# ajingu/RealSenseCalibration

Hardware: NVIDIA B200
Metric: LM iterations/sec (higher is better)
Workload: dtype f64

## Files before the change

realsensecalibration_b200/csrc/ba_cuda.cu:

```cuda
#include <dlfcn.h>

#include <algorithm>
#include <atomic>
#include <chrono>
#include <cmath>
#include <string>

#include "ba_dense.cuh"
#include "ba_dense_blocked.cuh"
#include "ba_kernels.cuh"
#include "ba_structure.cuh"
#include "ba_rcs.cuh"
#include "ba_fused_a.cuh"
#include "ba_strip_a.cuh"
#include "ba_exchange.cuh"
#include "ba_rig.cuh"

using namespace ba;

namespace {
typedef struct ncclComm* ncclComm_t;
struct NcclUniqueId { char internal[128]; };
struct Nccl {
  void* handle = nullptr;
// ... 479 lines not shown
  {
    FoldJob J = {{p->bp0.p, p->bp1.p, nullptr, nullptr}, {S_XE2, S_DE2, 0, 0}, {0, 0, 0, 0}};
    BA_LAUNCH(p, KT_FOLD, k_fold_multi, 2, 1024, 0, J, gce, p->scal.p);
  }
  BA_LAUNCH(p, KT_CANDIDATE, (k_candidate<6>), gcf, 256, 0, S.nf, p->f_act_ptr.p, p->xf.p, p->sf.p, p->yf.p, p->xf_c.p, p->bp0.p, p->bp1.p);
  {
    FoldJob J = {{p->bp0.p, p->bp1.p, nullptr, nullptr}, {S_XF2, S_DF2, 0, 0}, {0, 0, 0, 0}};
    BA_LAUNCH(p, KT_FOLD, k_fold_multi, 2, 1024, 0, J, gcf, p->scal.p);
  }
  BA_CUDA_TRY(cudaGetLastError());
  fam_end(p, F_UPDATE);
  fam_begin(p, F_COST);
  BA_TRY(run_cost_candidate(p));
  fam_end(p, F_COST);
  return allreduce_step_scalars(p);
}

FaParams fa_params(ba_cuda_problem* p, const ba_cuda_options& opt) {
  const Structure& S = p->S;
  FusedA& F = p->FA;
  const size_t nt = (size_t)F.n_tiles;
  FaParams P;
  P.tiles = F.tiles.p; P.e_ptr = S.e_ptr.p; P.ob_f = S.ob_f0.p; P.uv = p->uv.p;
  P.ob_meta = p->use_strip ? p->SA.ob_meta.p : F.ob_meta.p;
  P.tile_cams = p->use_strip ? p->SA.strip_cams.p : F.cams.group_target.p; P.cap = F.cap;
  P.pts_cap = F.pts_cap; P.tcam = F.tcam; P.tcs = F.tcs; P.pent_cap = F.pent_cap;
  P.pitem_begin = F.pairs.item_begin.p; P.pitem_end = F.pairs.item_end.p; P.pent = F.pairs.ent.p;
  P.citem_begin = F.cams.item_begin.p; P.citem_end = F.cams.item_end.p; P.cent = F.cams.ent.p;
  P.xe = p->xe.p; P.se = p->se.p; P.tab_f = p->tab_f.p; P.radius = p->scal.p + S_RADIUS;
  P.min_diag = opt.min_lm_diagonal; P.max_diag = opt.max_lm_diagonal;
  P.partP = F.partP.p; P.partC = F.partC.p; P.Lz = F.Lz.p; P.se_out = p->se.p;
  P.cost_partial = p->fa_part.p; P.g2_partial = p->fa_part.p + nt; P.gmax_partial = p->fa_part.p + 2 * nt;
  P.yf = p->yf.p; P.tabc_f = p->tabc_f.p; P.xe_c = p->xe_c.p;
  P.mcc_partial = p->fa_part.p + 3 * nt; P.x2_partial = p->fa_part.p + 4 * nt; P.d2_partial = p->fa_part.p + 5 * nt;
  P.cand_partial = p->fa_part.p + 6 * nt;
  P.RES = p->RES.p; P.JE = p->JE.p; P.JF = p->JF0.p;
  P.status = p->status.p;
  P.loss = p->loss;
  return P;
}

int fa_set_smem_attr(ba_cuda_problem* p) {
  if (!p->smem_attr_set) {
    const int kMax = (int)FA_SMEM_MAX;
    BA_CUDA_TRY(cudaFuncSetAttribute(k_fa_pass1<FA_FULL>, cudaFuncAttributeMaxDynamicSharedMemorySize, kMax));
    BA_CUDA_TRY(cudaFuncSetAttribute(k_fa_pass1<FA_NORMS>, cudaFuncAttributeMaxDynamicSharedMemorySize, kMax));
    BA_CUDA_TRY(cudaFuncSetAttribute(k_fa_pass1<FA_GRAD>, cudaFuncAttributeMaxDynamicSharedMemorySize, kMax));
    BA_CUDA_TRY(cudaFuncSetAttribute(k_fa_pass1<FA_FIRST>, cudaFuncAttributeMaxDynamicSharedMemorySize, kMax));
    BA_CUDA_TRY(cudaFuncSetAttribute(k_fa_pass2, cudaFuncAttributeMaxDynamicSharedMemorySize, kMax));
    BA_CUDA_TRY(cudaFuncSetAttribute(k_fa_jac, cudaFuncAttributeMaxDynamicSharedMemorySize, kMax));
    BA_CUDA_TRY(cudaFuncSetAttribute(k_sa_pass1<SA_FULL>, cudaFuncAttributeMaxDynamicSharedMemorySize, kMax));
    BA_CUDA_TRY(cudaFuncSetAttribute(k_sa_pass1<SA_GRAD>, cudaFuncAttributeMaxDynamicSharedMemorySize, kMax));
    BA_CUDA_TRY(cudaFuncSetAttribute(k_sa_pass1<SA_FIRST>, cudaFuncAttributeMaxDynamicSharedMemorySize, kMax));
    p->smem_attr_set = true;
  }
  return BA_OK;
}

int fa_reduce(ba_cuda_problem* p, bool cams, bool pairs) {
  const Structure& S = p->S;
  FusedA& F = p->FA;
  if (cams) {
    const ItemSet& I = F.cams;
    if (I.red_ch.n > 0)
      BA_LAUNCH(p, KT_FA_RED, (k_reduce_items<FA_NVC>), grid_for(I.red_ch.n, 4), 128, 0, I.red_ch.n, I.red_ch.ch, I.red_ch.seg.p, I.red_ch.begin.p,
                I.tgt_ptr.p, I.red_items.p, F.partC.p, F.red1C.p);
    BA_LAUNCH(p, KT_FA_RED, (k_reduce_final<FA_NVC>), grid_for(S.nf, 4), 128, 0, (int)S.nf, I.red_ch.seg_first.p, F.red1C.p, F.camacc.p);
  }
  if (pairs) {
    const ItemSet& I = F.pairs;
    if (I.red_ch.n > 0)
      BA_LAUNCH(p, KT_FA_RED, (k_reduce_items<36>), grid_for(I.red_ch.n, 4), 128, 0, I.red_ch.n, I.red_ch.ch, I.red_ch.seg.p, I.red_ch.begin.p,
                I.tgt_ptr.p, I.red_items.p, F.partP.p, F.red1P.p);
    BA_LAUNCH(p, KT_FA_RED, (k_reduce_final<36>), grid_for(S.ndest, 4), 128, 0, S.ndest, I.red_ch.seg_first.p, F.red1P.p, p->Pacc.p);
  }
  BA_CUDA_TRY(cudaGetLastError());
  return BA_OK;
}

int sa_linearize(ba_cuda_problem* p, const ba_cuda_options& opt, bool grad_only, bool first);

int fa_linearize(ba_cuda_problem* p, const ba_cuda_options& opt, bool norms, bool grad_only = false, bool first = false) {
  const Structure& S = p->S;
  FusedA& F = p->FA;
  BA_TRY(fa_set_smem_attr(p));
  if (p->use_strip) return sa_linearize(p, opt, grad_only, first);
  fam_begin(p, F_JAC);
  if (norms || first) {
    BA_LAUNCH(p, KT_MISC, k_fill, grid_for(S.nf * 6, 256), 256, 0, p->sf.p, S.nf * 6, 1.0);
    BA_LAUNCH(p, KT_MISC, k_fill, grid_for(S.ne * 3, 256), 256, 0, p->se.p, S.ne * 3, 1.0);
  }
  BA_TRY(build_tables(p, false));
  const FaParams P = fa_params(p, opt);
  const int nt = F.n_tiles;
  if (norms) {
    BA_LAUNCH(p, KT_FA_P1L, (k_fa_pass1<FA_NORMS>), nt, F.threads, F.smem1(), P);
    BA_TRY(fa_reduce(p, true, false));
    BA_TRY(allreduce(p, F.camacc.p, (size_t)S.nf * FA_NVC, kNcclSum));
    BA_LAUNCH(p, KT_MISC, (k_jacobi_scale<6, FA_NVC>), grid_for(S.nf * 6, 256), 256, 0, S.nf, F.camacc.p, p->sf.p);
    BA_CUDA_TRY(cudaGetLastError());
    fam_end(p, F_JAC);
    return BA_OK;
  }
  BA_CUDA_TRY(cudaMemsetAsync(p->status.p, 0, sizeof(int), p->st));
  if (grad_only) BA_LAUNCH(p, KT_FA_P1L, (k_fa_pass1<FA_GRAD>), nt, F.threads, F.smem1(), P);
  else if (first) BA_LAUNCH(p, KT_FA_P1, (k_fa_pass1<FA_FIRST>), nt, F.threads, F.smem1(), P);
// ... 124 lines not shown
  const double* radius = p->scal.p + S_RADIUS;
  const bool pcg = p->solver == BA_RCS_PCG;
  const bool sx = sx_active(p);
  fam_begin(p, F_SCHUR);
  if (pcg && sx) {
  } else if (pcg) {
    if (p->world > 1) BA_CUDA_TRY(cudaMemsetAsync(p->Sb.p, 0, p->Sb.bytes(), p->st));
    BA_LAUNCH(p, KT_ASSEMBLE, k_assemble_bsr, grid_for((int64_t)S.ndest * 36, 256), 256, 0, S.ndest, p->R.l2g.p, p->Pacc.p, nullptr, p->Sb.p);
  } else {
    BA_CUDA_TRY(cudaMemsetAsync(p->Sd.p, 0, sizeof(double) * n * n, p->st));
    BA_LAUNCH(p, KT_ASSEMBLE, k_assemble_dense, grid_for((int64_t)S.ndest * 36, 256), 256, 0, S.ndest, S.dest_fa.p, S.dest_fb.p, p->Pacc.p,
              nullptr, n, p->Sd.p);
  }
  fam_end(p, F_SCHUR);
  if (p->world > 1 && !(pcg && sx)) {
    fam_begin(p, F_COLL);
    if (pcg) BA_TRY(allreduce(p, p->Sb.p, (size_t)p->R.nd * 36, kNcclSum));
    else BA_TRY(allreduce(p, p->Sd.p, n * n, kNcclSum));
    fam_end(p, F_COLL);
  }
  fam_begin(p, F_SOLVE);
  if (pcg) {
    if (p->use_strip)
      BA_LAUNCH(p, KT_ASSEMBLE, k_sa_diag_rhs_bsr, grid_for(S.nf * 6, 128), 128, 0, S.nf, p->R.diag.p, F.camacc.p, radius, opt.min_lm_diagonal,
                opt.max_lm_diagonal, p->Sb.p, p->rhs.p);
    else
      BA_LAUNCH(p, KT_ASSEMBLE, k_diag_rhs_bsr, grid_for(S.nf * 6, 128), 128, 0, S.nf, p->R.diag.p, F.camacc.p, FA_NVC, F.camacc.p + 27, FA_NVC,
                radius, opt.min_lm_diagonal, opt.max_lm_diagonal, p->Sb.p, p->rhs.p);
    {
      LaunchScope scope(p, KT_RCS);
      BA_TRY(launch_pcg(p->pcg, p->R, p->Sb.p, p->rhs.p, p->yf.p, p->status.p, opt, p->st));
    }
    BA_CUDA_TRY(cudaMemcpyAsync(&p->h_pcg_iters, p->pcg.iters.p, sizeof(int), cudaMemcpyDeviceToHost, p->st));
  } else {
    if (p->use_strip)
      BA_LAUNCH(p, KT_ASSEMBLE, k_sa_diag_rhs_dense, grid_for(S.nf * 6, 128), 128, 0, S.nf, F.camacc.p, radius, opt.min_lm_diagonal,
                opt.max_lm_diagonal, n, p->Sd.p, p->rhs.p);
    else
      BA_LAUNCH(p, KT_ASSEMBLE, k_diag_rhs_dense, grid_for(S.nf * 6, 128), 128, 0, S.nf, F.camacc.p, FA_NVC, F.camacc.p + 27, FA_NVC, radius,
                opt.min_lm_diagonal, opt.max_lm_diagonal, n, p->Sd.p, p->rhs.p);
    LaunchScope scope(p, KT_RCS);
    BA_TRY(dense_solve(p, n));
  }
  fam_end(p, F_SOLVE);
  fam_begin(p, F_UPDATE);
  const int gcf = (int)grid_for(S.nf * 6, 256);
  BA_LAUNCH(p, KT_CANDIDATE, (k_candidate<6>), gcf, 256, 0, S.nf, p->f_act_ptr.p, p->xf.p, p->sf.p, p->yf.p, p->xf_c.p, p->bp0.p, p->bp1.p);
  {
    FoldJob J = {{p->bp0.p, p->bp1.p, nullptr, nullptr}, {S_XF2, S_DF2, 0, 0}, {0, 0, 0, 0}};
    BA_LAUNCH(p, KT_FOLD, k_fold_multi, 2, 1024, 0, J, gcf, p->scal.p);
  }
  BA_TRY(build_tables(p, true));
  const FaParams P = fa_params(p, opt);
  BA_LAUNCH(p, KT_FA_P2, k_fa_pass2, F.n_tiles, F.threads2, F.smem2(), P);
  {
    FoldJob J = {{P.mcc_partial, P.x2_partial, P.d2_partial, P.cand_partial}, {S_MCC, S_XE2, S_DE2, S_CAND}, {0, 0, 0, 0}};
    BA_LAUNCH(p, KT_FOLD, k_fold_multi, 4, 1024, 0, J, F.n_tiles, p->scal.p);
  }
  BA_CUDA_TRY(cudaGetLastError());
  fam_end(p, F_UPDATE);
  return allreduce_step_scalars(p);
}

bool lm_fused(const ba_cuda_problem* p) { return p->model == 0 && p->use_fused && !p->lm.opt.force_generic_path; }

int sx_prepare(ba_cuda_problem* p) {
  const Structure& S = p->S;
  SparseExchange& X = p->SX;
  X.on = false; X.world = p->world; X.nvc = p->use_strip ? SA_NVC : FA_NVC;
  if (!nccl().AllGather || !env_int("BA_SX", 0, 1, 1)) return BA_OK;
  cudaStream_t st = p->st;
  const int64_t nf = S.nf, nd = p->R.nd;
  DVec<int32_t> cflag, cpos, dflag, dpos;
  BA_TRY(cflag.alloc(nf + 1)); BA_TRY(cpos.alloc(nf + 1)); BA_TRY(dflag.alloc((size_t)S.ndest + 1)); BA_TRY(dpos.alloc((size_t)S.ndest + 1));
  BA_CUDA_TRY(cudaMemsetAsync(cflag.p, 0, sizeof(int32_t) * (nf + 1), st));
  BA_CUDA_TRY(cudaMemsetAsync(dflag.p, 0, sizeof(int32_t) * ((size_t)S.ndest + 1), st));
  k_sx_flags<<<grid_for(nf, 256), 256, 0, st>>>(S.fobs_ptr.p, nf, cflag.p);
  k_sx_send_flags<<<grid_for(S.ndest, 256), 256, 0, st>>>(S.ndest, S.dest_fa.p, S.dest_fb.p, cflag.p, dflag.p);
  BA_TRY(cub_call([&](void* t, size_t& b) { return cub::DeviceScan::ExclusiveSum(t, b, cflag.p, cpos.p, (int)(nf + 1), st); }));
  BA_TRY(cub_call([&](void* t, size_t& b) { return cub::DeviceScan::ExclusiveSum(t, b, dflag.p, dpos.p, S.ndest + 1, st); }));
  int32_t h2[2] = {0, 0};
  BA_CUDA_TRY(cudaMemcpyAsync(&h2[0], cpos.p + nf, sizeof(int32_t), cudaMemcpyDeviceToHost, st));
  BA_CUDA_TRY(cudaMemcpyAsync(&h2[1], dpos.p + S.ndest, sizeof(int32_t), cudaMemcpyDeviceToHost, st));
  BA_CUDA_TRY(cudaStreamSynchronize(st));
  X.nc_local = h2[0]; X.n_send = h2[1];
  BA_TRY(X.my_cams.alloc((size_t)X.nc_local)); BA_TRY(X.send_d.alloc((size_t)X.n_send));
  k_sx_compact<<<grid_for(nf, 256), 256, 0, st>>>(cflag.p, cpos.p, nf, X.my_cams.p);
  k_sx_compact<<<grid_for(S.ndest, 256), 256, 0, st>>>(dflag.p, dpos.p, S.ndest, X.send_d.p);
  DVec<int64_t> cnt;
  BA_TRY(cnt.alloc(2 * (size_t)p->world));
  const int64_t mine[2] = {X.n_send, X.nc_local};
  BA_CUDA_TRY(cudaMemcpyAsync(cnt.p + 2 * p->rank, mine, sizeof(mine), cudaMemcpyHostToDevice, st));
  int rc = nccl().AllGather(cnt.p + 2 * p->rank, cnt.p, 2, kNcclInt64, p->comm, st);
  if (rc != 0) return fail(BA_ERR_NCCL, "ncclAllGather failed (%d)", rc);
  std::vector<int64_t> h(2 * (size_t)p->world);
  BA_CUDA_TRY(cudaMemcpyAsync(h.data(), cnt.p, sizeof(int64_t) * h.size(), cudaMemcpyDeviceToHost, st));
  BA_CUDA_TRY(cudaStreamSynchronize(st));
  int64_t sum_nd = 0, max_nd = 1, max_nc = 1;
  for (int r = 0; r < p->world; ++r) { sum_nd += h[2 * r]; max_nd = std::max(max_nd, h[2 * r]); max_nc = std::max(max_nc, h[2 * r + 1]); }
  if ((double)max_nd * p->world > 1.5 * (double)nd) return BA_OK;
  X.max_nd = (int)max_nd; X.max_nc = (int)max_nc;
  X.slot = (size_t)max_nd * 36 + (size_t)max_nc * X.nvc + 4;
  DVec<int32_t> lists_d, lists_c;
  BA_TRY(lists_d.alloc((size_t)max_nd * p->world)); BA_TRY(lists_c.alloc((size_t)max_nc * p->world));
  BA_CUDA_TRY(cudaMemsetAsync(lists_d.p, 0xff, sizeof(int32_t) * (size_t)max_nd * p->world, st));
  BA_CUDA_TRY(cudaMemsetAsync(lists_c.p, 0xff, sizeof(int32_t) * (size_t)max_nc * p->world, st));
  k_sx_gather_l2g<<<grid_for(X.n_send, 256), 256, 0, st>>>(X.n_send, X.send_d.p, p->R.l2g.p, lists_d.p + (size_t)max_nd * p->rank);
  BA_CUDA_TRY(cudaMemcpyAsync(lists_c.p + (size_t)max_nc * p->rank, X.my_cams.p, sizeof(int32_t) * X.nc_local, cudaMemcpyDeviceToDevice, st));
  rc = nccl().AllGather(lists_d.p + (size_t)max_nd * p->rank, lists_d.p, (size_t)max_nd, kNcclInt32, p->comm, st);
  if (rc == 0) rc = nccl().AllGather(lists_c.p + (size_t)max_nc * p->rank, lists_c.p, (size_t)max_nc, kNcclInt32, p->comm, st);
// ... 1307 lines not shown
```

realsensecalibration_b200/csrc/ba_fused_a.cuh:

```cuda
#pragma once
#include <cuda_pipeline.h>

#include <chrono>
#include <cstdio>

#include "ba_kernels.cuh"
#include "ba_structure.cuh"

namespace ba {

constexpr int FA_TOBS_DEFAULT = 256;
constexpr int FA_KMAX = 64;
constexpr int FA_TPTS = 4096;
constexpr int FA_TCAM = 48;
constexpr int FA_CH_PAIR = 16;
constexpr int FA_CH_RED = 64;
constexpr int FA_NVC = 33;
constexpr int FA_MAX_THREADS = 512;
constexpr int FA_THREADS_DEFAULT = 128;
constexpr int FA_REC = 22;
constexpr int FA_REC2 = 10;
constexpr int FA_PENT_MAX = 6144;
constexpr size_t FA_SMEM_MAX = 231000;
constexpr int FA_LS = 10;
// ... 427 lines not shown
                                                          sb, keys.p, vals.p);
      L.lap("pair fill (32-bit keys)");
      D.mode = 1; D.sb = sb; D.key_bits = 2 * sb + tb;
      D.tile_cam_ptr = F.cams.tile_group_ptr.p; D.tile_cams = F.cams.group_target.p;
      D.dh_keys = S.dh_keys.p; D.dh_val = S.dh_val.p; D.dh_mask = S.dh_mask; D.dh_shift = S.dh_shift;
      BA_TRY(build_items<uint32_t>(F.pairs, keys, vals, np, F.n_tiles, S.ndest, F.ch_pair, true, D, st));
    } else {
      DVec<uint64_t> keys;
      BA_TRY(keys.alloc(np));
      k_fa_pair_fill<<<grid_for(ne, 128), 128, 0, st>>>(S.e_ptr.p, S.ob_f0.p, ne, nf, off.p, tile_of_pt.p, F.tile_pt_ptr.p, S.dest_keys.p,
                                                        S.ndest, S.dh_keys.n ? S.dh_keys.p : nullptr, S.dh_val.p, S.dh_mask, S.dh_shift, keys.p,
                                                        vals.p);
      L.lap("pair fill");
      D.key_bits = bits_for((uint64_t)F.n_tiles * (uint64_t)S.ndest);
      BA_TRY(build_items<uint64_t>(F.pairs, keys, vals, np, F.n_tiles, S.ndest, F.ch_pair, true, D, st));
    }
  }
  {
    const int nt = F.n_tiles;
    BA_TRY(F.tile_pent_ptr.alloc((size_t)nt + 1)); BA_TRY(F.tile_cent_ptr.alloc((size_t)nt + 1));
    k_fa_tile_ent_ptr<<<grid_for(nt + 1, 256), 256, 0, st>>>(nt, F.pairs.tile_group_ptr.p, F.pairs.group_ptr.p, F.tile_pent_ptr.p);
    k_fa_tile_ent_ptr<<<grid_for(nt + 1, 256), 256, 0, st>>>(nt, F.cams.tile_group_ptr.p, F.cams.group_ptr.p, F.tile_cent_ptr.p);
    DVec<int> stat;
    BA_TRY(stat.alloc_zero(3, st));
    k_fa_tile_stats<<<grid_for(nt, 256), 256, 0, st>>>(nt, F.tile_pt_ptr.p, F.cams.tile_group_ptr.p, F.tile_pent_ptr.p, stat.p);
    int h[3] = {0, 0, 0};
    BA_CUDA_TRY(cudaMemcpyAsync(h, stat.p, sizeof(h), cudaMemcpyDeviceToHost, st));
    BA_CUDA_TRY(cudaStreamSynchronize(st));
    F.pts_cap = std::max(1, std::min(h[0], FA_TPTS));
    F.tcam = std::max(1, std::min(h[1], FA_TCAM));
    F.tcs = F.tcam | 1;
    F.pent_cap = std::min(h[2], FA_PENT_MAX);
    F.pent_cap += F.pent_cap & 1;
    if (F.smem1() > FA_SMEM_MAX) {
      const size_t excess = (F.smem1() - FA_SMEM_MAX + 7) / 8 * 2;
      F.pent_cap = (size_t)F.pent_cap > excess ? F.pent_cap - (int)excess : 0;
    }
    if (F.smem1() > FA_SMEM_MAX || F.smem2() > FA_SMEM_MAX || F.smemj(FA_JAC_THREADS) > FA_SMEM_MAX) return BA_ERR_UNSUPPORTED;
  }
  L.lap("pair items, geometry");
  BA_TRY(F.tiles.alloc((size_t)F.n_tiles));
  k_fa_tile_desc<<<grid_for(F.n_tiles, 256), 256, 0, st>>>(F.n_tiles, F.tile_pt_ptr.p, S.e_ptr.p, F.cams.tile_group_ptr.p, F.tile_pent_ptr.p,
                                                          F.tile_cent_ptr.p, F.pairs.tile_item_ptr.p, F.cams.tile_item_ptr.p, F.tiles.p);
  BA_TRY(F.partP.alloc((size_t)F.pairs.n_items * 36)); BA_TRY(F.partC.alloc((size_t)F.cams.n_items * FA_NVC));
  BA_TRY(F.red1P.alloc((size_t)F.pairs.red_ch.n * 36)); BA_TRY(F.red1C.alloc((size_t)F.cams.red_ch.n * FA_NVC));
  BA_TRY(F.camacc.alloc((size_t)nf * FA_NVC + 2 + 64));
  BA_TRY(F.Lz.alloc((size_t)ne * 9));
  BA_CUDA_TRY(cudaStreamSynchronize(st));
  BA_CUDA_TRY(cudaGetLastError());
  F.ready = true;
  return BA_OK;
}

__device__ __forceinline__ void fa_linearize(const double* __restrict__ T, const double* X, const double* s, double2 ob, double* r,
                                             double* je, double* jf) {
  double q[3];
  mat3_vec(T, X, q);
  const double p0 = q[0] + T[18], p1 = q[1] + T[19], p2 = q[2] + T[20];
  r[0] = T[21] * p0 / p2 + T[23] - ob.x;
  r[1] = T[22] * p1 / p2 + T[24] - ob.y;
  const double iz = 1.0 / p2;
  const double a = T[21] * iz, bb = -T[21] * p0 * iz * iz, cc = T[22] * iz, dd = -T[22] * p1 * iz * iz;
  double D[9];
  rot_deriv(T + 9, T[25] != 0.0 ? X : q, D);
#pragma unroll
  for (int k = 0; k < 3; ++k) {
    jf[k] = (a * D[k] + bb * D[6 + k]) * T[26 + k];
    jf[6 + k] = (cc * D[3 + k] + dd * D[6 + k]) * T[26 + k];
  }
  jf[3] = a * T[29]; jf[4] = 0.0;        jf[5] = bb * T[31];
  jf[9] = 0.0;       jf[10] = cc * T[30]; jf[11] = dd * T[31];
  je[0] = (a * T[0] + bb * T[6]) * s[0]; je[1] = (a * T[1] + bb * T[7]) * s[1]; je[2] = (a * T[2] + bb * T[8]) * s[2];
  je[3] = (cc * T[3] + dd * T[6]) * s[0]; je[4] = (cc * T[4] + dd * T[7]) * s[1]; je[5] = (cc * T[5] + dd * T[8]) * s[2];
}

__device__ __forceinline__ bool fa_chol3(const double* M , double* Lp) {
  const double d0 = M[0];
  if (!(d0 > 0.0) || !isfinite(d0)) return false;
  const double i0 = rsqrt(d0);
  const double l10 = M[1] * i0, l20 = M[2] * i0;
  const double d1 = M[3] - l10 * l10;
  if (!(d1 > 0.0) || !isfinite(d1)) return false;
  const double i1 = rsqrt(d1);
  const double l21 = (M[4] - l20 * l10) * i1;
  const double d2 = M[5] - l20 * l20 - l21 * l21;
  if (!(d2 > 0.0) || !isfinite(d2)) return false;
  Lp[0] = l10; Lp[1] = l20; Lp[2] = l21; Lp[3] = i0; Lp[4] = i1; Lp[5] = rsqrt(d2);
  return true;
}
__device__ __forceinline__ void fa_fwd3(const double* Lp, double* x) {
  x[0] *= Lp[3];
  x[1] = (x[1] - Lp[0] * x[0]) * Lp[4];
  x[2] = (x[2] - Lp[1] * x[0] - Lp[2] * x[1]) * Lp[5];
}
__device__ __forceinline__ void fa_bwd3(const double* Lp, double* x) {
  x[2] *= Lp[5];
  x[1] = (x[1] - Lp[2] * x[2]) * Lp[4];
  x[0] = (x[0] - Lp[0] * x[1] - Lp[1] * x[2]) * Lp[3];
}

struct FaParams {
  const FaTile* tiles;
  const int64_t* e_ptr; const int32_t* ob_f; const uint32_t* ob_meta; const double2* uv;
  const int32_t* tile_cams;
  const int64_t* pitem_begin; const int64_t* pitem_end; const int32_t* pent;
  const int64_t* citem_begin; const int64_t* citem_end; const int32_t* cent;
  int cap, pts_cap, tcam, tcs, pent_cap;
  const double* xe; const double* se; const double* tab_f; const double* radius;
  double min_diag, max_diag;
  double* partP; double* partC; double* Lz; double* se_out;
  double* cost_partial; double* gmax_partial; double* g2_partial;
  const double* yf; const double* tabc_f; double* xe_c;
  double* mcc_partial; double* x2_partial; double* d2_partial; double* cand_partial;
  double* RES; double* JE; double* JF;
  int* status;
  LossSpec loss;
};

__device__ __forceinline__ double fa_apply_loss(const LossSpec L, double* r, double* je, double* jf) {
  const double s = r[0] * r[0] + r[1] * r[1];
  if (L.type == 0) return s;
  double rho, w;
  loss_apply(L, s, &rho, &w);
  r[0] *= w; r[1] *= w;
#pragma unroll
  for (int k = 0; k < 6; ++k) je[k] *= w;
// ... 593 lines not shown
```

realsensecalibration_b200/csrc/ba_strip_a.cuh:

```cuda
#pragma once
#include "ba_fused_a.cuh"

namespace ba {

constexpr int SA_NT = 512;
constexpr int SA_NCS_MAX = 64;
constexpr int SA_NVC = 39;
constexpr int SA_REC = 22;
constexpr int SA_NF_CAP = 1024;
constexpr int SA_POS_MAX = 4096;
constexpr int SA_CM_MAX = 8;
constexpr int SA_TYPE_IDLE = 0, SA_TYPE_PAIR = 1, SA_TYPE_FLUSH = 2, SA_TYPE_CAM = 3;
constexpr int SA_FULL = 0, SA_GRAD = 2, SA_FIRST = 3;

__host__ __device__ inline int sa_xs_len(int pts_cap) { return (3 * pts_cap + 4 + 1) & ~1; }

struct __align__(16) SaTile {
  int64_t pt0, ob0, pos0, ent0, pidx0, fout0;
  int32_t npts, nobs, npos, nent;
};
static_assert(sizeof(SaTile) == 64, "SaTile is loaded as four 16-byte words");
struct __align__(16) SaStrip {
  int64_t cam0, pout0, cout0;
  int32_t tile0, ntiles, ncs, nflush;
  int32_t flush_t0;
  int32_t npp, ncact, cbase;
};
static_assert(sizeof(SaStrip) == 64, "SaStrip");

struct StripA {
  bool ready = false;
  int n_tiles = 0, n_strips = 0, tobs = 0, L = 0, kmax = 0;
  int cap_pos = 0, pts_cap = 0, ncs_cap = 0, tcs = 0, ent_cap = 0, pidx_cap = 0, segw = 0, nobs_cap = 0;
  int64_t n_pout = 0, n_fout = 0, n_cout = 0;
  DVec<int64_t> tile_pt_ptr;
  DVec<SaTile> tiles;
  DVec<SaStrip> strips;
  DVec<int32_t> strip_cams;
  DVec<int64_t> strip_cam_ptr;
  DVec<uint32_t> slot_out;
  DVec<uint32_t> pm;
  DVec<double2> puv;
  DVec<uint16_t> pidx;
  DVec<int32_t> ent;
  DVec<uint16_t> seg;
  DVec<uint32_t> ob_meta;
  DVec<int32_t> red_items_p, red_items_c;
  DVec<int64_t> tgt_ptr_p, tgt_ptr_c;
  Chunks red_ch_p, red_ch_c;
  DVec<double> partP, partC, red1P, red1C;
  size_t smem() const {
    size_t b = ((size_t)cap_pos * SA_REC + (size_t)tcs * TAB + 2 * (size_t)sa_xs_len(pts_cap)) * 8;
    b += (size_t)cap_pos * 16 + (size_t)cap_pos * 4 + (size_t)pidx_cap * 2 + (size_t)ent_cap * 4 + (size_t)segw * 2 + 64;
    return b;
  }
};

__global__ void k_sa_strip_keys(int64_t nb, const int32_t* __restrict__ ob_e, const int32_t* __restrict__ ob_f,
                                const int32_t* __restrict__ tile_of_pt, int L, int64_t nf, uint64_t* __restrict__ keys) {
  const int64_t o = blockIdx.x * (int64_t)blockDim.x + threadIdx.x;
  if (o < nb) keys[o] = (uint64_t)(tile_of_pt[ob_e[o]] / L) * (uint64_t)nf + (uint64_t)ob_f[o];
}
__global__ void k_sa_split_keys(int ng, const uint64_t* __restrict__ ukeys, int64_t nf, int32_t* __restrict__ gstrip, int32_t* __restrict__ gcam) {
  const int g = blockIdx.x * blockDim.x + threadIdx.x;
  if (g >= ng) return;
  gstrip[g] = (int32_t)(ukeys[g] / (uint64_t)nf);
  gcam[g] = (int32_t)(ukeys[g] % (uint64_t)nf);
}
__global__ void k_sa_obs_slot(int64_t nb, const int32_t* __restrict__ ob_e, const int32_t* __restrict__ ob_f,
                              const int32_t* __restrict__ tile_of_pt, const int64_t* __restrict__ tile_pt_ptr, int L,
                              const int64_t* __restrict__ strip_cam_ptr, const int32_t* __restrict__ strip_cams,
                              uint8_t* __restrict__ ob_slot, uint32_t* __restrict__ ob_meta) {
  const int64_t o = blockIdx.x * (int64_t)blockDim.x + threadIdx.x;
  if (o >= nb) return;
  const int32_t e = ob_e[o], tile = tile_of_pt[e], strip = tile / L, cam = ob_f[o];
  int64_t lo = strip_cam_ptr[strip], hi = strip_cam_ptr[strip + 1];
  const int64_t c0 = lo;
  while (lo < hi) {
    const int64_t mid = (lo + hi) >> 1;
    if (strip_cams[mid] < cam) lo = mid + 1; else hi = mid;
  }
  const uint32_t slot = (uint32_t)min((int64_t)255, lo - c0);
  ob_slot[o] = (uint8_t)slot;
  ob_meta[o] = (uint32_t)(e - tile_pt_ptr[tile]) | (slot << 16);
}

__device__ __forceinline__ int sa_class(int ncs, int slot, int l) { return ncs >= 8 ? (slot & 7) : (l & 7); }
__device__ __forceinline__ int sa_class_rows(int nobs, int max_class) { return min(max_class, (nobs * 17 / 16 + 7) / 8); }

__global__ void __launch_bounds__(256)
k_sa_tile_sizes(int n_tiles, int L, const int64_t* __restrict__ tile_pt_ptr, const int64_t* __restrict__ e_ptr,
                const uint8_t* __restrict__ ob_slot, const int64_t* __restrict__ strip_cam_ptr, int64_t* __restrict__ tile_npos,
                int64_t* __restrict__ tile_nent, int64_t* __restrict__ tile_npidx, int* __restrict__ stat) {
  __shared__ int cls[8];
  __shared__ int npair, dup;
  const int t = blockIdx.x;
  if (threadIdx.x < 8) cls[threadIdx.x] = 0;
  if (threadIdx.x == 0) { npair = 0; dup = 0; }
  __syncthreads();
  const int64_t pt0 = tile_pt_ptr[t], pt1 = tile_pt_ptr[t + 1];
  const int64_t ob0 = e_ptr[pt0];
  const int nobs = (int)(e_ptr[pt1] - ob0), npts = (int)(pt1 - pt0);
  const int strip = t / L;
  const int ncs = (int)(strip_cam_ptr[strip + 1] - strip_cam_ptr[strip]);
  for (int l = threadIdx.x; l < nobs; l += blockDim.x) atomicAdd(&cls[sa_class(ncs, ob_slot[ob0 + l], l)], 1);
  for (int lp = threadIdx.x; lp < npts; lp += blockDim.x) {
    const int64_t b = e_ptr[pt0 + lp], n = e_ptr[pt0 + lp + 1];
// ... 662 lines not shown
  A.ent_cap = max_nent;
  if (A.smem() > FA_SMEM_MAX) {
    const size_t excess = (A.smem() - FA_SMEM_MAX + 15) / 16 * 4;
    if ((size_t)A.ent_cap <= excess) return BA_ERR_UNSUPPORTED;
    A.ent_cap = (int)(A.ent_cap - excess) & ~3;
    if (A.ent_cap < max_nent / 2) return BA_ERR_UNSUPPORTED;
  }
  BA_TRY(A.ent.alloc((size_t)tot[1] + 8)); BA_TRY(A.seg.alloc((size_t)nt * A.segw + 8));
  DVec<int64_t> t_nfl, fout0;
  BA_TRY(t_nfl.alloc_zero((size_t)nt + 1, st));
  {
    SaEntParams P;
    P.L = L; P.ncs_cap = A.ncs_cap; P.segw = A.segw; P.stage_cap = 12288;
    P.tiles = A.tiles.p; P.strips = A.strips.p; P.e_ptr = S.e_ptr.p; P.ob_e = S.ob_e.p; P.ob_slot = ob_slot.p; P.pidx = A.pidx.p;
    P.dslot = dslot.p; P.cslot = cslot.p; P.cthr = cthr.p; P.thr_of = thr_of.p; P.ent = A.ent.p; P.seg = A.seg.p; P.tile_nfl = t_nfl.p;
    const size_t sm = ((size_t)2 * A.segw + 1 + P.stage_cap) * sizeof(int);
    BA_CUDA_TRY(cudaFuncSetAttribute(k_sa_tile_entries, cudaFuncAttributeMaxDynamicSharedMemorySize, 100 * 1024));
    k_sa_tile_entries<<<nt, 512, sm, st>>>(P);
  }
  BA_TRY(sa_exclusive_scan(t_nfl, fout0, nt + 1, st));
  k_sa_set_fout<<<grid_for(nt, 256), 256, 0, st>>>(nt, fout0.p, A.tiles.p);
  BA_CUDA_TRY(cudaMemcpyAsync(&A.n_fout, fout0.p + nt, sizeof(int64_t), cudaMemcpyDeviceToHost, st));
  BA_CUDA_TRY(cudaStreamSynchronize(st));
  BA_CUDA_TRY(cudaGetLastError());
  Lp.lap("strip: entries");
  const int64_t n_pblocks = A.n_pout + A.n_fout;
  if (n_pblocks >= (int64_t)INT32_MAX / 64 || A.n_cout >= (int64_t)INT32_MAX / 64) return BA_ERR_UNSUPPORTED;
  {
    DVec<int32_t> ptarget, ctarget, iota;
    BA_TRY(ptarget.alloc((size_t)n_pblocks)); BA_TRY(ctarget.alloc((size_t)A.n_cout));
    k_sa_targets_persist<<<grid_for((int64_t)ns * SA_NT, 256), 256, 0, st>>>(ns, A.strips.p, A.slot_out.p, slot_dest.p, A.strip_cams.p, nf,
                                                                            S.dh_keys.p, S.dh_val.p, S.dh_mask, S.dh_shift, ptarget.p, ctarget.p);
    k_sa_targets_flush<<<grid_for(nt, 4), 128, 0, st>>>(nt, L, A.segw, nf_cap, A.tiles.p, A.strips.p, A.seg.p, fl_dest.p, A.strip_cams.p, nf,
                                                       S.dh_keys.p, S.dh_val.p, S.dh_mask, S.dh_shift, A.n_pout, ptarget.p);
    const int64_t nmax = std::max(n_pblocks, A.n_cout);
    BA_TRY(iota.alloc((size_t)nmax));
    k_iota<<<grid_for(nmax, 256), 256, 0, st>>>(iota.p, nmax, 0);
    BA_TRY(sort_to_csr(ptarget.p, iota.p, n_pblocks, S.ndest, A.tgt_ptr_p, A.red_items_p, st));
    BA_TRY(build_chunks(A.red_ch_p, A.tgt_ptr_p.p, S.ndest, FA_CH_RED, st));
    BA_TRY(sort_to_csr(ctarget.p, iota.p, A.n_cout, nf, A.tgt_ptr_c, A.red_items_c, st));
    BA_TRY(build_chunks(A.red_ch_c, A.tgt_ptr_c.p, (int)nf, FA_CH_RED, st));
    BA_CUDA_TRY(cudaStreamSynchronize(st));
  }
  Lp.lap("strip: reduction lists");
  BA_TRY(A.partP.alloc((size_t)n_pblocks * 36)); BA_TRY(A.partC.alloc((size_t)A.n_cout * SA_NVC));
  BA_TRY(A.red1P.alloc((size_t)A.red_ch_p.n * 36)); BA_TRY(A.red1C.alloc((size_t)A.red_ch_c.n * SA_NVC));
  F.n_tiles = nt; F.tobs = tobs; F.kmax = A.kmax; F.cap = std::max(A.nobs_cap, 1);
  F.threads = SA_NT; F.threads2 = env_int("BA_FA_THREADS2", 32, FA_MAX_THREADS, tobs >= 640 ? 256 : 128) / 32 * 32;
  F.pts_cap = A.pts_cap; F.tcam = std::min(A.ncs_cap, FA_TCAM); F.tcs = F.tcam | 1; F.pent_cap = 0;
  if (F.smem2() > FA_SMEM_MAX || F.smemj(FA_JAC_THREADS) > FA_SMEM_MAX) return BA_ERR_UNSUPPORTED;
  BA_TRY(F.tiles.alloc((size_t)nt));
  k_sa_fa_tiles<<<grid_for(nt, 256), 256, 0, st>>>(nt, L, A.tiles.p, A.strips.p, F.tiles.p);
  BA_TRY(F.camacc.alloc((size_t)nf * SA_NVC + 2 + 64));
  BA_TRY(F.Lz.alloc((size_t)ne * 9));
  BA_CUDA_TRY(cudaStreamSynchronize(st));
  BA_CUDA_TRY(cudaGetLastError());
  if (Lp.on)
    std::fprintf(stderr, "[ba_cuda timing]   strip geometry: tobs %d L %d tiles %d strips %d | positions %d points %d cameras %d entries staged %d of %d "
                         "owner slots %d | smem %zu B | blocks: %lld per strip + %lld flushed, %lld camera\n", tobs, L, nt, ns, A.cap_pos, A.pts_cap,
                 A.ncs_cap, A.ent_cap, max_nent, A.segw, A.smem(), (long long)A.n_pout, (long long)A.n_fout, (long long)A.n_cout);
  A.ready = true; F.ready = true;
  return BA_OK;
}

struct SaParams {
  const SaStrip* strips; const SaTile* tiles; const int32_t* strip_cams; const uint32_t* slot_out;
  const uint32_t* pm; const double2* puv; const uint16_t* pidx; const int32_t* ent; const uint16_t* seg;
  int segw, cap_pos, pts_cap, tcs, ent_cap, pidx_cap;
  const double* xe; const double* se; const double* tab_f; const double* radius;
  double min_diag, max_diag;
  double* partP; double* partC; int64_t n_pout;
  double* Lz; double* se_out; double* cost_partial; double* g2_partial; double* gmax_partial; int* status;
  int dbg;
  unsigned long long* clocks;
  LossSpec loss;
};

__device__ __forceinline__ uint32_t sa_smem_u32(const void* p) { return (uint32_t)__cvta_generic_to_shared(p); }
__device__ __forceinline__ void sa_mbar_init(uint64_t* bar, int count) {
  asm volatile("mbarrier.init.shared::cta.b64 [%0], %1;" ::"r"(sa_smem_u32(bar)), "r"(count) : "memory");
}
__device__ __forceinline__ void sa_mbar_expect_tx(uint64_t* bar, uint32_t bytes) {
  asm volatile("mbarrier.arrive.expect_tx.shared::cta.b64 _, [%0], %1;" ::"r"(sa_smem_u32(bar)), "r"(bytes) : "memory");
}
__device__ __forceinline__ void sa_mbar_wait(uint64_t* bar, uint32_t parity) {
  uint32_t ok = 0;
  const uint32_t a = sa_smem_u32(bar);
  do {
    asm volatile("{\n .reg .pred p;\n mbarrier.try_wait.parity.shared::cta.b64 p, [%1], %2;\n selp.u32 %0, 1, 0, p;\n}\n"
                 : "=r"(ok) : "r"(a), "r"(parity) : "memory");
  } while (!ok);
}
__device__ __forceinline__ void sa_bulk_g2s(void* dst, const void* src, uint32_t bytes, uint64_t* bar) {
  asm volatile("cp.async.bulk.shared::cluster.global.mbarrier::complete_tx::bytes [%0], [%1], %2, [%3];"
               ::"r"(sa_smem_u32(dst)), "l"(src), "r"(bytes), "r"(sa_smem_u32(bar)) : "memory");
}

template <int MODE>
__global__ void __launch_bounds__(SA_NT, 1) k_sa_pass1(SaParams P) {
  constexpr bool FIRST = MODE == SA_FIRST, FULL = MODE == SA_FULL || FIRST, UNIT = FIRST;
  extern __shared__ __align__(128) double smem[];
  double* rec = smem;
  double* tabs = rec + (size_t)P.cap_pos * SA_REC;
  double* xs = tabs + (size_t)P.tcs * TAB;
  double* ss = xs + sa_xs_len(P.pts_cap);
  double2* puv_s = reinterpret_cast<double2*>(ss + sa_xs_len(P.pts_cap));
  uint32_t* pm_s = reinterpret_cast<uint32_t*>(puv_s + P.cap_pos);
  uint16_t* pidx_s = reinterpret_cast<uint16_t*>(pm_s + P.cap_pos);
  int32_t* ent_s = reinterpret_cast<int32_t*>(pidx_s + P.pidx_cap);
  uint16_t* seg_s = reinterpret_cast<uint16_t*>(ent_s + P.ent_cap);
  uint64_t* bars = reinterpret_cast<uint64_t*>(seg_s + P.segw);
  __shared__ double red[96];
  const int tid = threadIdx.x, lane = tid & 31, warp = tid >> 5;
// ... 317 lines not shown
  const int64_t t = blockIdx.x * (int64_t)blockDim.x + threadIdx.x;
  if (t >= nf * SA_NVC) return;
  const int64_t c = t / SA_NVC;
  const int v = (int)(t % SA_NVC);
  double f;
  if (v < 21) {
    int a = 0, rem = v;
    while (rem >= 6 - a) { rem -= 6 - a; ++a; }
    f = sf[6 * c + a] * sf[6 * c + a + rem];
  } else if (v < 33) {
    f = sf[6 * c + (v - 21) % 6];
  } else {
    f = sf[6 * c + (v - 33)] * sf[6 * c + (v - 33)];
  }
  camacc[t] *= f;
}
__global__ void k_sa_jacobi_scale(int64_t nf, const double* __restrict__ camacc, double* __restrict__ sf) {
  const int64_t t = blockIdx.x * (int64_t)blockDim.x + threadIdx.x;
  if (t >= nf * 6) return;
  sf[t] = 1.0 / (1.0 + sqrt(camacc[(t / 6) * SA_NVC + 33 + (t % 6)]));
}
__global__ void k_sa_diag_rhs_bsr(int64_t nf, const int32_t* __restrict__ diag, const double* __restrict__ camacc, const double* __restrict__ radius_p,
                                  double min_diag, double max_diag, double* __restrict__ Sb, double* __restrict__ rhs) {
  const int64_t t = blockIdx.x * (int64_t)blockDim.x + threadIdx.x;
  if (t >= nf * 6) return;
  const int64_t f = t / 6;
  const int a = (int)(t % 6);
  const double* H = camacc + f * SA_NVC;
  double* B = Sb + (int64_t)diag[f] * 36;
#pragma unroll
  for (int b = 0; b < 6; ++b) {
    double h = H[a <= b ? sym_idx6(a, b) : sym_idx6(b, a)];
    if (a == b) { const double d = sqrt(fmin(fmax(H[33 + a], min_diag), max_diag) / *radius_p); h += d * d; }
    B[a * 6 + b] += h;
  }
  rhs[t] = H[21 + a] - H[27 + a];
}
__global__ void k_sa_diag_rhs_dense(int64_t nf, const double* __restrict__ camacc, const double* __restrict__ radius_p, double min_diag,
                                    double max_diag, int64_t n, double* __restrict__ Sd, double* __restrict__ rhs) {
  const int64_t t = blockIdx.x * (int64_t)blockDim.x + threadIdx.x;
  if (t >= nf * 6) return;
  const int64_t f = t / 6;
  const int a = (int)(t % 6);
  const double* H = camacc + f * SA_NVC;
#pragma unroll
  for (int b = 0; b < 6; ++b) {
    double h = H[a <= b ? sym_idx6(a, b) : sym_idx6(b, a)];
    if (a == b) { const double d = sqrt(fmin(fmax(H[33 + a], min_diag), max_diag) / *radius_p); h += d * d; }
    Sd[(6 * f + a) * n + 6 * f + b] += h;
  }
  rhs[t] = H[21 + a] - H[27 + a];
}

}
```

Before: 118.6.

## Add strip-based pass-2 kernel with double-buffered bulk async tile loads

Adds a new k_sa_pass2 kernel that runs the post-solve candidate pass per strip instead of per tile. Camera tables are staged once per strip and tile inputs are prefetched with bulk async copies into double buffers. The aim is to reuse the camera tables across tiles and overlap global loads with compute, replacing the per-tile k_fa_pass2 launch. It is gated by BA_SA_P2 (default on) and a shared-memory size check. It adds complexity and the risk of fewer, larger blocks with one block per SM, which lowers parallelism.

```diff
diff --git a/realsensecalibration_b200/csrc/ba_cuda.cu b/realsensecalibration_b200/csrc/ba_cuda.cu
--- a/realsensecalibration_b200/csrc/ba_cuda.cu
+++ b/realsensecalibration_b200/csrc/ba_cuda.cu
@@ -555,6 +555,7 @@
     BA_CUDA_TRY(cudaFuncSetAttribute(k_sa_pass1<SA_FULL>, cudaFuncAttributeMaxDynamicSharedMemorySize, kMax));
     BA_CUDA_TRY(cudaFuncSetAttribute(k_sa_pass1<SA_GRAD>, cudaFuncAttributeMaxDynamicSharedMemorySize, kMax));
     BA_CUDA_TRY(cudaFuncSetAttribute(k_sa_pass1<SA_FIRST>, cudaFuncAttributeMaxDynamicSharedMemorySize, kMax));
+    BA_CUDA_TRY(cudaFuncSetAttribute(k_sa_pass2, cudaFuncAttributeMaxDynamicSharedMemorySize, kMax));
     p->smem_attr_set = true;
   }
   return BA_OK;
@@ -785,10 +786,41 @@
   }
   BA_TRY(build_tables(p, true));
   const FaParams P = fa_params(p, opt);
-  BA_LAUNCH(p, KT_FA_P2, k_fa_pass2, F.n_tiles, F.threads2, F.smem2(), P);
+  int n_part = F.n_tiles;
+  if (p->use_strip && p->SA.p2) {
+    const StripA& A = p->SA;
+    Sa2Params Q;
+    Q.strips = A.strips.p; Q.tiles = A.tiles.p; Q.strip_cams = A.strip_cams.p;
+    Q.pm = A.pm.p; Q.puv = A.puv.p; Q.pidx = A.pidx.p;
+    Q.cap_pos = A.cap_pos; Q.pts_cap = A.pts_cap; Q.tcs = A.tcs; Q.pidx_cap = A.pidx_cap;
+    Q.xe = p->xe.p; Q.se = p->se.p; Q.Lz = F.Lz.p; Q.tab_f = p->tab_f.p; Q.tabc_f = p->tabc_f.p; Q.yf = p->yf.p;
+    Q.xe_c = p->xe_c.p;
+    Q.mcc_partial = P.mcc_partial; Q.x2_partial = P.x2_partial; Q.d2_partial = P.d2_partial; Q.cand_partial = P.cand_partial;
+    Q.loss = p->loss;
+    static DVec<unsigned long long>* clk = nullptr;
+    Q.clocks = nullptr;
+    if (env_int("BA_SA_CLOCKS", 0, 1, 0)) {
+      if (!clk) { clk = new DVec<unsigned long long>(); BA_TRY(clk->alloc(8)); }
+      BA_CUDA_TRY(cudaMemsetAsync(clk->p, 0, 8 * sizeof(unsigned long long), p->st));
+      Q.clocks = clk->p;
+    }
+    BA_LAUNCH(p, KT_FA_P2, k_sa_pass2, A.n_strips, SA2_NT, A.smem2(), Q);
+    if (Q.clocks) {
+      unsigned long long h[8];
+      BA_CUDA_TRY(cudaMemcpyAsync(h, Q.clocks, sizeof(h), cudaMemcpyDeviceToHost, p->st));
+      BA_CUDA_TRY(cudaStreamSynchronize(p->st));
+      const double n = (double)A.n_tiles;
+      std::fprintf(stderr, "[ba_cuda clocks] pass 2, cycles per tile as thread 0 sees them: top %.0f | wait inputs %.0f | observations + barrier %.0f | "
+                           "points + barrier %.0f | candidate (own) %.0f | barrier after candidate %.0f | sum %.0f\n", h[0] / n, h[1] / n, h[2] / n,
+                   h[3] / n, h[4] / n, h[5] / n, (h[0] + h[1] + h[2] + h[3] + h[4] + h[5]) / n);
+    }
+    n_part = A.n_strips;
+  } else {
+    BA_LAUNCH(p, KT_FA_P2, k_fa_pass2, F.n_tiles, F.threads2, F.smem2(), P);
+  }
   {
     FoldJob J = {{P.mcc_partial, P.x2_partial, P.d2_partial, P.cand_partial}, {S_MCC, S_XE2, S_DE2, S_CAND}, {0, 0, 0, 0}};
-    BA_LAUNCH(p, KT_FOLD, k_fold_multi, 4, 1024, 0, J, F.n_tiles, p->scal.p);
+    BA_LAUNCH(p, KT_FOLD, k_fold_multi, 4, 1024, 0, J, n_part, p->scal.p);
   }
   BA_CUDA_TRY(cudaGetLastError());
   fam_end(p, F_UPDATE);
diff --git a/realsensecalibration_b200/csrc/ba_fused_a.cuh b/realsensecalibration_b200/csrc/ba_fused_a.cuh
--- a/realsensecalibration_b200/csrc/ba_fused_a.cuh
+++ b/realsensecalibration_b200/csrc/ba_fused_a.cuh
@@ -503,26 +503,39 @@
   return BA_OK;
 }
 
+template <typename TF>
+__device__ __forceinline__ void fa_linearize_f(const TF& T, const double* X, const double* s, double2 ob, double* r, double* je, double* jf) {
+  double q[3];
+  q[0] = T(0) * X[0] + T(1) * X[1] + T(2) * X[2];
+  q[1] = T(3) * X[0] + T(4) * X[1] + T(5) * X[2];
+  q[2] = T(6) * X[0] + T(7) * X[1] + T(8) * X[2];
+  const double p0 = q[0] + T(18), p1 = q[1] + T(19), p2 = q[2] + T(20);
+  r[0] = T(21) * p0 / p2 + T(23) - ob.x;
+  r[1] = T(22) * p1 / p2 + T(24) - ob.y;
+  const double iz = 1.0 / p2;
+  const double a = T(21) * iz, bb = -T(21) * p0 * iz * iz, cc = T(22) * iz, dd = -T(22) * p1 * iz * iz;
+  const double* b = T(25) != 0.0 ? X : q;
+  double D[9];
+#pragma unroll
+  for (int k = 0; k < 3; ++k) {
+    const double a0 = T(9 + k), a1 = T(12 + k), a2 = T(15 + k);
+    D[k] = a1 * b[2] - a2 * b[1];
+    D[3 + k] = a2 * b[0] - a0 * b[2];
+    D[6 + k] = a0 * b[1] - a1 * b[0];
+  }
+#pragma unroll
+  for (int k = 0; k < 3; ++k) {
+    jf[k] = (a * D[k] + bb * D[6 + k]) * T(26 + k);
+    jf[6 + k] = (cc * D[3 + k] + dd * D[6 + k]) * T(26 + k);
+  }
+  jf[3] = a * T(29); jf[4] = 0.0;        jf[5] = bb * T(31);
+  jf[9] = 0.0;       jf[10] = cc * T(30); jf[11] = dd * T(31);
+  je[0] = (a * T(0) + bb * T(6)) * s[0]; je[1] = (a * T(1) + bb * T(7)) * s[1]; je[2] = (a * T(2) + bb * T(8)) * s[2];
+  je[3] = (cc * T(3) + dd * T(6)) * s[0]; je[4] = (cc * T(4) + dd * T(7)) * s[1]; je[5] = (cc * T(5) + dd * T(8)) * s[2];
+}
 __device__ __forceinline__ void fa_linearize(const double* __restrict__ T, const double* X, const double* s, double2 ob, double* r,
                                              double* je, double* jf) {
-  double q[3];
-  mat3_vec(T, X, q);
-  const double p0 = q[0] + T[18], p1 = q[1] + T[19], p2 = q[2] + T[20];
-  r[0] = T[21] * p0 / p2 + T[23] - ob.x;
-  r[1] = T[22] * p1 / p2 + T[24] - ob.y;
-  const double iz = 1.0 / p2;
-  const double a = T[21] * iz, bb = -T[21] * p0 * iz * iz, cc = T[22] * iz, dd = -T[22] * p1 * iz * iz;
-  double D[9];
-  rot_deriv(T + 9, T[25] != 0.0 ? X : q, D);
-#pragma unroll
-  for (int k = 0; k < 3; ++k) {
-    jf[k] = (a * D[k] + bb * D[6 + k]) * T[26 + k];
-    jf[6 + k] = (cc * D[3 + k] + dd * D[6 + k]) * T[26 + k];
-  }
-  jf[3] = a * T[29]; jf[4] = 0.0;        jf[5] = bb * T[31];
-  jf[9] = 0.0;       jf[10] = cc * T[30]; jf[11] = dd * T[31];
-  je[0] = (a * T[0] + bb * T[6]) * s[0]; je[1] = (a * T[1] + bb * T[7]) * s[1]; je[2] = (a * T[2] + bb * T[8]) * s[2];
-  je[3] = (cc * T[3] + dd * T[6]) * s[0]; je[4] = (cc * T[4] + dd * T[7]) * s[1]; je[5] = (cc * T[5] + dd * T[8]) * s[2];
+  fa_linearize_f([&](int f) { return T[f]; }, X, s, ob, r, je, jf);
 }
 
 __device__ __forceinline__ bool fa_chol3(const double* M , double* Lp) {
diff --git a/realsensecalibration_b200/csrc/ba_strip_a.cuh b/realsensecalibration_b200/csrc/ba_strip_a.cuh
--- a/realsensecalibration_b200/csrc/ba_strip_a.cuh
+++ b/realsensecalibration_b200/csrc/ba_strip_a.cuh
@@ -13,7 +13,11 @@
 constexpr int SA_TYPE_IDLE = 0, SA_TYPE_PAIR = 1, SA_TYPE_FLUSH = 2, SA_TYPE_CAM = 3;
 constexpr int SA_FULL = 0, SA_GRAD = 2, SA_FIRST = 3;
 
+constexpr int SA2_NT = 512;
+constexpr int SA2_REC = 10;
+
 __host__ __device__ inline int sa_xs_len(int pts_cap) { return (3 * pts_cap + 4 + 1) & ~1; }
+__host__ __device__ inline int sa_lz_len(int pts_cap) { return (9 * pts_cap + 2 + 1) & ~1; }
 
 struct __align__(16) SaTile {
   int64_t pt0, ob0, pos0, ent0, pidx0, fout0;
@@ -53,6 +57,11 @@
     size_t b = ((size_t)cap_pos * SA_REC + (size_t)tcs * TAB + 2 * (size_t)sa_xs_len(pts_cap)) * 8;
     b += (size_t)cap_pos * 16 + (size_t)cap_pos * 4 + (size_t)pidx_cap * 2 + (size_t)ent_cap * 4 + (size_t)segw * 2 + 64;
     return b;
+  }
+  bool p2 = false;
+  size_t smem2() const {
+    const size_t buf = ((size_t)cap_pos * 2 + 2 * (size_t)sa_xs_len(pts_cap) + (size_t)sa_lz_len(pts_cap)) * 8 + (size_t)cap_pos * 4 + (size_t)pidx_cap * 2;
+    return ((size_t)tcs * (TAB + 16 + 6) + (size_t)cap_pos * SA2_REC) * 8 + 2 * buf + 16;
   }
 };
 
@@ -821,13 +830,15 @@
   BA_TRY(F.tiles.alloc((size_t)nt));
   k_sa_fa_tiles<<<grid_for(nt, 256), 256, 0, st>>>(nt, L, A.tiles.p, A.strips.p, F.tiles.p);
   BA_TRY(F.camacc.alloc((size_t)nf * SA_NVC + 2 + 64));
-  BA_TRY(F.Lz.alloc((size_t)ne * 9));
+  BA_TRY(F.Lz.alloc_zero((size_t)ne * 9 + 2, st));
+  A.p2 = env_int("BA_SA_P2", 0, 1, 1) != 0 && A.smem2() <= FA_SMEM_MAX;
   BA_CUDA_TRY(cudaStreamSynchronize(st));
   BA_CUDA_TRY(cudaGetLastError());
   if (Lp.on)
     std::fprintf(stderr, "[ba_cuda timing]   strip geometry: tobs %d L %d tiles %d strips %d | positions %d points %d cameras %d entries staged %d of %d "
-                         "owner slots %d | smem %zu B | blocks: %lld per strip + %lld flushed, %lld camera\n", tobs, L, nt, ns, A.cap_pos, A.pts_cap,
-                 A.ncs_cap, A.ent_cap, max_nent, A.segw, A.smem(), (long long)A.n_pout, (long long)A.n_fout, (long long)A.n_cout);
+                         "owner slots %d | smem %zu B, pass 2 %zu B (%s) | blocks: %lld per strip + %lld flushed, %lld camera\n", tobs, L, nt, ns,
+                 A.cap_pos, A.pts_cap, A.ncs_cap, A.ent_cap, max_nent, A.segw, A.smem(), A.smem2(), A.p2 ? "strips" : "tiles", (long long)A.n_pout,
+                 (long long)A.n_fout, (long long)A.n_cout);
   A.ready = true; F.ready = true;
   return BA_OK;
 }
@@ -1251,4 +1262,211 @@
   rhs[t] = H[21 + a] - H[27 + a];
 }
 
-}
+struct Sa2Params {
+  const SaStrip* strips; const SaTile* tiles; const int32_t* strip_cams;
+  const uint32_t* pm; const double2* puv; const uint16_t* pidx;
+  int cap_pos, pts_cap, tcs, pidx_cap;
+  const double* xe; const double* se; const double* Lz; const double* tab_f; const double* tabc_f; const double* yf;
+  double* xe_c;
+  double* mcc_partial; double* x2_partial; double* d2_partial; double* cand_partial;
+  unsigned long long* clocks;
+  LossSpec loss;
+};
+
+__global__ void __launch_bounds__(SA2_NT, 1) k_sa_pass2(Sa2Params P) {
+  extern __shared__ __align__(128) double smem[];
+  double* tabs = smem;
+  double* tabc = tabs + (size_t)P.tcs * TAB;
+  double* yfs = tabc + (size_t)P.tcs * 16;
+  double* rec = yfs + (size_t)P.tcs * 6;
+  const int xs_len = sa_xs_len(P.pts_cap), lz_len = sa_lz_len(P.pts_cap);
+  double* bufd = rec + (size_t)P.cap_pos * SA2_REC;
+  const size_t bstride = (size_t)2 * P.cap_pos + 2 * (size_t)xs_len + lz_len;
+  uint32_t* bufi = reinterpret_cast<uint32_t*>(bufd + 2 * bstride);
+  const size_t istride = (size_t)P.cap_pos + (size_t)P.pidx_cap / 2;
+  uint64_t* bars = reinterpret_cast<uint64_t*>(bufi + 2 * istride);
+  __shared__ double red[128];
+  const int tid = threadIdx.x, lane = tid & 31, warp = tid >> 5;
+  const SaStrip S = P.strips[blockIdx.x];
+  const bool producer = tid == SA2_NT - 1;
+
+  auto buffers = [&](int b, double2*& puv_s, double*& xs, double*& ss, double*& lz, uint32_t*& pm_s, uint16_t*& pidx_s) {
+    double* d = bufd + (size_t)b * bstride;
+    puv_s = reinterpret_cast<double2*>(d); xs = d + 2 * (size_t)P.cap_pos; ss = xs + xs_len; lz = ss + xs_len;
+    pm_s = bufi + (size_t)b * istride; pidx_s = reinterpret_cast<uint16_t*>(pm_s + P.cap_pos);
+  };
+  auto issue = [&](const SaTile& T, int b) {
+    double2* puv_s; double *xs, *ss, *lz; uint32_t* pm_s; uint16_t* pidx_s;
+    buffers(b, puv_s, xs, ss, lz, pm_s, pidx_s);
+    const uint32_t b_uv = (uint32_t)T.npos * 16u, b_pm = (uint32_t)T.npos * 4u;
+    const uint32_t b_idx = (uint32_t)(((T.nobs + 7) & ~7) + ((T.npts + 1 + 7) & ~7)) * 2u;
+    const int64_t x0 = (3 * T.pt0) & ~(int64_t)1, z0 = (9 * T.pt0) & ~(int64_t)1;
+    const uint32_t b_x = (uint32_t)((3 * T.pt0 + 3 * T.npts - x0 + 1) & ~(int64_t)1) * 8u;
+    const uint32_t b_z = (uint32_t)((9 * T.pt0 + 9 * T.npts - z0 + 1) & ~(int64_t)1) * 8u;
+    asm volatile("fence.proxy.async.shared::cta;" ::: "memory");
+    sa_mbar_expect_tx(bars + b, b_uv + b_pm + b_idx + 2 * b_x + b_z);
+    sa_bulk_g2s(puv_s, P.puv + T.pos0, b_uv, bars + b);
+    sa_bulk_g2s(pm_s, P.pm + T.pos0, b_pm, bars + b);
+    sa_bulk_g2s(pidx_s, P.pidx + T.pidx0, b_idx, bars + b);
+    sa_bulk_g2s(xs, P.xe + x0, b_x, bars + b);
+    sa_bulk_g2s(ss, P.se + x0, b_x, bars + b);
+    sa_bulk_g2s(lz, P.Lz + z0, b_z, bars + b);
+  };
+
+  if (tid == 0) {
+    sa_mbar_init(bars + 0, 1);
+    sa_mbar_init(bars + 1, 1);
+    asm volatile("fence.mbarrier_init.release.cluster;" ::: "memory");
+  }
+  {
+    uint32_t* pt = reinterpret_cast<uint32_t*>(tabs);
+    uint32_t* pc = reinterpret_cast<uint32_t*>(tabc);
+    uint32_t* py = reinterpret_cast<uint32_t*>(yfs);
+    for (int s = warp; s < S.ncs; s += SA2_NT / 32) {
+      const int32_t cam = __ldg(P.strip_cams + S.cam0 + s);
+      const uint32_t* src = reinterpret_cast<const uint32_t*>(P.tab_f + (int64_t)TAB * cam + lane);
+      __pipeline_memcpy_async(pt + (size_t)(2 * lane) * P.tcs + s, src, 4);
+      __pipeline_memcpy_async(pt + (size_t)(2 * lane + 1) * P.tcs + s, src + 1, 4);
+      if (lane < 16) {
+        const uint32_t* sc = reinterpret_cast<const uint32_t*>(P.tabc_f + (int64_t)TAB * cam + kFaCandFields[lane]);
+        __pipeline_memcpy_async(pc + (size_t)(2 * lane) * P.tcs + s, sc, 4);
+        __pipeline_memcpy_async(pc + (size_t)(2 * lane + 1) * P.tcs + s, sc + 1, 4);
+      } else if (lane < 22) {
+        const int k = lane - 16;
+        const uint32_t* sy = reinterpret_cast<const uint32_t*>(P.yf + 6 * (int64_t)cam + k);
+        __pipeline_memcpy_async(py + (size_t)(2 * k) * P.tcs + s, sy, 4);
+        __pipeline_memcpy_async(py + (size_t)(2 * k + 1) * P.tcs + s, sy + 1, 4);
+      }
+    }
+    __pipeline_commit();
+    __pipeline_wait_prior(0);
+  }
+  __syncthreads();
+  SaTile Tn;
+  auto load_desc = [&](int tile) {
+    const int4* s4 = reinterpret_cast<const int4*>(P.tiles + tile);
+    int4* d4 = reinterpret_cast<int4*>(&Tn);
+#pragma unroll
+    for (int k = 0; k < 4; ++k) d4[k] = __ldg(s4 + k);
+  };
+  load_desc(S.tile0);
+  if (producer) issue(Tn, 0);
+  double mcc = 0.0, x2 = 0.0, d2 = 0.0, sq = 0.0;
+  uint32_t phase = 0;
+  long long ck[6] = {0, 0, 0, 0, 0, 0}, c_last = clock64();
+  auto tick = [&](int k) { if (P.clocks && tid == 0) { const long long c = clock64(); ck[k] += c - c_last; c_last = c; } };
+  for (int ti = 0; ti < S.ntiles; ++ti) {
+    const int b = ti & 1;
+    const SaTile T = Tn;
+    if (ti + 1 < S.ntiles) load_desc(S.tile0 + ti + 1);
+    double2* puv_s; double *xs, *ss, *lz; uint32_t* pm_s; uint16_t* pidx_s;
+    buffers(b, puv_s, xs, ss, lz, pm_s, pidx_s);
+    const int npos = T.npos, npts = T.npts;
+    const int xoff = (int)((3 * T.pt0) & 1), zoff = (int)((9 * T.pt0) & 1);
+    const uint16_t* pbeg = pidx_s + ((T.nobs + 7) & ~7);
+    tick(0);
+    sa_mbar_wait(bars + b, (phase >> b) & 1u); phase ^= 1u << b;
+    tick(1);
+    for (int pos = tid; pos < npos; pos += SA2_NT) {
+      const uint32_t m = pm_s[pos];
+      if (!(m >> 31)) continue;
+      const int lp = (int)(m & 0xfffu), slot = (int)((m >> 12) & 0x3fu);
+      const double X[3] = {xs[xoff + 3 * lp], xs[xoff + 3 * lp + 1], xs[xoff + 3 * lp + 2]};
+      const double s[3] = {ss[xoff + 3 * lp], ss[xoff + 3 * lp + 1], ss[xoff + 3 * lp + 2]};
+      double r[2], je[6], jf[12];
+      fa_linearize_f([&](int f) { return fa_table_field(tabs, P.tcs, f, slot); }, X, s, puv_s[pos], r, je, jf);
+      fa_apply_loss(P.loss, r, je, jf);
+      double q0 = 0.0, q1 = 0.0;
+#pragma unroll
+      for (int k = 0; k < 6; ++k) {
+        const double y = fa_table_field(yfs, P.tcs, k, slot);
+        q0 += jf[k] * y; q1 += jf[6 + k] * y;
+      }
+      double2* R2 = reinterpret_cast<double2*>(rec + (size_t)pos * SA2_REC);
+#pragma unroll
+      for (int k = 0; k < 3; ++k) R2[k] = make_double2(je[2 * k], je[2 * k + 1]);
+      R2[3] = make_double2(r[0], r[1]);
+      R2[4] = make_double2(q0, q1);
+    }
+    __syncthreads();
+    tick(2);
+    if (producer && ti + 1 < S.ntiles) issue(Tn, b ^ 1);
+    for (int base = 0; base < npts; base += SA2_NT / 4) {
+      const int lp = base + (tid >> 2), q = tid & 3;
+      const bool on = lp < npts;
+      int l0 = 0, l1 = 0;
+      double Lp[6] = {0.0, 0.0, 0.0, 1.0, 1.0, 1.0}, t[3] = {0.0, 0.0, 0.0};
+      if (on) {
+        l0 = pbeg[lp]; l1 = pbeg[lp + 1];
+        const double* in = lz + zoff + 9 * lp;
+#pragma unroll
+        for (int k = 0; k < 6; ++k) Lp[k] = in[k];
+      }
+      for (int l = l0 + q; l < l1; l += 4) {
+        const double* R = rec + (size_t)pidx_s[l] * SA2_REC;
+#pragma unroll
+        for (int rr = 0; rr < 2; ++rr) {
+          double u[3] = {R[3 * rr], R[3 * rr + 1], R[3 * rr + 2]};
+          fa_fwd3(Lp, u);
+          const double qv = R[8 + rr];
+          t[0] -= u[0] * qv; t[1] -= u[1] * qv; t[2] -= u[2] * qv;
+        }
+      }
+#pragma unroll
+      for (int k = 0; k < 3; ++k) { t[k] += __shfl_xor_sync(0xffffffffu, t[k], 1); t[k] += __shfl_xor_sync(0xffffffffu, t[k], 2); }
+      if (!on) continue;
+      {
+        const double* in = lz + zoff + 9 * lp;
+        t[0] += in[6]; t[1] += in[7]; t[2] += in[8];
+      }
+      fa_bwd3(Lp, t);
+      for (int l = l0 + q; l < l1; l += 4) {
+        const double* R = rec + (size_t)pidx_s[l] * SA2_REC;
+#pragma unroll
+        for (int rr = 0; rr < 2; ++rr) {
+          const double m = -(R[3 * rr] * t[0] + R[3 * rr + 1] * t[1] + R[3 * rr + 2] * t[2]) - R[8 + rr];
+          mcc += m * (R[6 + rr] + m / 2.0);
+        }
+      }
+      if (q < 3) {
+        const int k = q;
+        const double tk = k == 0 ? t[0] : (k == 1 ? t[1] : t[2]);
+        const double xv = xs[xoff + 3 * lp + k];
+        const double c = xv + (-(tk) * ss[xoff + 3 * lp + k]);
+        P.xe_c[3 * (T.pt0 + lp) + k] = c;
+        xs[xoff + 3 * lp + k] = c;
+        if (l1 > l0) { x2 += xv * xv; const double d = xv - c; d2 += d * d; }
+      }
+    }
+    __syncthreads();
+    tick(3);
+    for (int pos = tid; pos < npos; pos += SA2_NT) {
+      const uint32_t m = pm_s[pos];
+      if (!(m >> 31)) continue;
+      const int lp = (int)(m & 0xfffu), slot = (int)((m >> 12) & 0x3fu);
+      const double2 ob = puv_s[pos];
+      auto C = [&](int f) { return fa_table_field(tabc, P.tcs, f, slot); };
+      const double X[3] = {xs[xoff + 3 * lp], xs[xoff + 3 * lp + 1], xs[xoff + 3 * lp + 2]};
+      const double q0 = C(0) * X[0] + C(1) * X[1] + C(2) * X[2];
+      const double q1 = C(3) * X[0] + C(4) * X[1] + C(5) * X[2];
+      const double q2 = C(6) * X[0] + C(7) * X[1] + C(8) * X[2];
+      const double p0 = q0 + C(9), p1 = q1 + C(10), p2 = q2 + C(11);
+      const double r0 = C(12) * p0 / p2 + C(14) - ob.x;
+      const double r1 = C(13) * p1 / p2 + C(15) - ob.y;
+      double sc = r0 * r0 + r1 * r1;
+      if (P.loss.type != 0) { double w; loss_apply(P.loss, sc, &sc, &w); }
+      sq += sc;
+    }
+    tick(4);
+    __syncthreads();
+    tick(5);
+  }
+  if (P.clocks && tid == 0)
+    for (int k = 0; k < 6; ++k) atomicAdd(P.clocks + k, (unsigned long long)ck[k]);
+  double v[4] = {mcc, x2, d2, sq};
+  const bool mx[4] = {false, false, false, false};
+  fa_block_reduce(v, mx, 4, red);
+  if (tid == 0) { P.mcc_partial[blockIdx.x] = v[0]; P.x2_partial[blockIdx.x] = v[1]; P.d2_partial[blockIdx.x] = v[2]; P.cand_partial[blockIdx.x] = v[3]; }
+}
+
+}
```

Result: no change. 119.4, median of 6 (+0.7%).
